# duongve13112002/DiffusionSpatialControl

Measured on AMD Instinct MI355X. Metric: 512x512 images/sec, SD1.5 25-step DPM++2M Karras with region-biased cross-attention, higher is better.
Workload: dtype f16; 1 GPU; SD1.5 512x512, 25-step DPM++2M Karras, CFG 7.5, 2 region masks, 1 image(s) per generation, 2 generation(s) in flight per GPU; images_per_gpu=1, parallelism=dp1 (independent images, no per-step collective), hip_graph=True, outputs_finite=True, full=False

## Files before the change

### diffusionspatialcontrol_amd/_lib.py

```python
import ctypes
import os
import re

_HERE = os.path.dirname(os.path.abspath(__file__))
_LIB = None


class DscLibraryError(RuntimeError):
    pass


def lib_path():
    return os.environ.get("DSC_LIB_PATH") or os.path.join(_HERE, "libdsc_hip.so")


def header_path():
    return os.path.join(os.path.dirname(_HERE), "include", "dsc_hip.h")


def declared_symbols():
    txt = open(header_path()).read()
    txt = re.sub(r"/\*.*?\*/", "", txt, flags=re.S)
    return sorted(set(re.findall(r"\b(dsc_[a-z0-9_]+)\s*\(", txt)))

# ... 34 lines not shown
    "dsc_cfg_linear_step_rows": (ctypes.c_int, [_vp, _vp, _vp, ctypes.c_int, _vp, _vp, _vp, _vp, ctypes.c_int, ctypes.c_int,
                                 _vp, ctypes.c_int, ctypes.c_int, ctypes.c_int, _vp]),
    "dsc_cfg_linear_step_rows_rescale": (ctypes.c_int, [_vp, _vp, _vp, ctypes.c_int, _vp, _vp, _vp, _vp, ctypes.c_int,
                                         ctypes.c_int, _vp, _vp, ctypes.c_int, ctypes.c_int, ctypes.c_int, _vp]),
    "dsc_dpmpp2m_update": (ctypes.c_int, [_vp, _vp, _vp] + [ctypes.c_float] * 3 + [_vp, ctypes.c_int64, ctypes.c_int, _vp]),
    "dsc_groupnorm_workspace_bytes": (ctypes.c_size_t, [ctypes.c_int] * 4),
    "dsc_groupnorm_silu": (ctypes.c_int, [_vp] * 4 + [ctypes.c_int] * 4 + [ctypes.c_float, ctypes.c_int, ctypes.c_int,
                                                                             _vp, ctypes.c_size_t, _vp]),
    "dsc_groupnorm_nhwc_workspace_bytes": (ctypes.c_size_t, [ctypes.c_int] * 4),
    "dsc_debug_set_gn_mode": (None, [ctypes.c_int]),
    "dsc_groupnorm_silu_nhwc": (ctypes.c_int, [_vp] * 5 + [ctypes.c_int64] + [ctypes.c_int] * 4 +
                                [ctypes.c_float, ctypes.c_int, ctypes.c_int, _vp, ctypes.c_size_t, _vp]),
    "dsc_groupnorm_silu_nhwc_cat": (ctypes.c_int, [_vp, _vp, ctypes.c_int] + [_vp] * 5 + [ctypes.c_int64] + [ctypes.c_int] * 4 +
                                    [ctypes.c_float, ctypes.c_int, ctypes.c_int, _vp, ctypes.c_size_t, _vp]),
    "dsc_set_workspace_slot": (ctypes.c_int, [ctypes.c_int]),
    "dsc_set_tuning_profile": (ctypes.c_int, [ctypes.c_int]),
    "dsc_get_tuning_profile": (ctypes.c_int, []),
    "dsc_linear_lt_stats": (None, [_vp]),
    "dsc_has_library_gemm": (ctypes.c_int, []),
    "dsc_add_bias_residual": (ctypes.c_int, [_vp] * 4 + [ctypes.c_int64, ctypes.c_int, ctypes.c_int, _vp]),
    "dsc_linear_f16": (ctypes.c_int, [_vp] * 5 + [ctypes.c_int64, ctypes.c_int, ctypes.c_int] + [ctypes.c_int64] * 3 +
                       [ctypes.c_int, ctypes.c_int, _vp]),
    "dsc_debug_set_conv_stamps": (None, [_vp]),
    "dsc_debug_set_conv_ring": (None, [ctypes.c_int]),
    "dsc_conv3x3_supported": (ctypes.c_int, [ctypes.c_int] * 5),
    "dsc_conv3x3_workspace_bytes": (ctypes.c_size_t, [ctypes.c_int] * 6),
    "dsc_conv3x3_nhwc_f16": (ctypes.c_int, [_vp] * 5 + [ctypes.c_int] * 5 + [ctypes.c_int64] * 3 +
                             [ctypes.c_int, ctypes.c_int, ctypes.c_int, ctypes.c_int, _vp, ctypes.c_size_t, _vp]),
    "dsc_conv3x3_up2x_pack_f16": (ctypes.c_int, [_vp, _vp, ctypes.c_int, ctypes.c_int, _vp]),
    "dsc_conv3x3_up2x_supported": (ctypes.c_int, [ctypes.c_int] * 5),
    "dsc_conv3x3_up2x_workspace_bytes": (ctypes.c_size_t, [ctypes.c_int] * 6),
    "dsc_conv3x3_up2x_nhwc_f16": (ctypes.c_int, [_vp] * 4 + [ctypes.c_int] * 6 + [_vp, ctypes.c_size_t, ctypes.c_int64, ctypes.c_int64,
                                                                                   ctypes.c_int, _vp]),
    "dsc_conv3x3_fewcin_f16": (ctypes.c_int, [_vp] * 4 + [ctypes.c_int] * 6 + [_vp]),
    "dsc_linear_lt_f16": (ctypes.c_int, [_vp] * 5 + [ctypes.c_int64, ctypes.c_int, ctypes.c_int] + [ctypes.c_int64] * 3 +
                          [ctypes.c_int, _vp]),
    "dsc_linear_rows_f16": (ctypes.c_int, [_vp] * 4 + [ctypes.c_int] * 3 + [ctypes.c_int64] * 2 + [ctypes.c_int, ctypes.c_int, _vp]),
    "dsc_linear_ln_f16": (ctypes.c_int, [_vp] * 5 + [ctypes.c_int64, ctypes.c_int, ctypes.c_int] + [ctypes.c_int64] * 3 +
                          [ctypes.c_int, _vp, ctypes.c_int, _vp, ctypes.c_float, _vp, ctypes.c_int, _vp]),
    "dsc_debug_set_gemm_stages": (None, [ctypes.c_int]),
    "dsc_linear_qkv_f16": (ctypes.c_int, [_vp] * 5 + [ctypes.c_int64, ctypes.c_int, ctypes.c_int, ctypes.c_int64, ctypes.c_int64,
                                          ctypes.c_int, ctypes.c_int, _vp, ctypes.c_int, _vp, ctypes.c_float, ctypes.c_int, _vp]),
    "dsc_add_layernorm": (ctypes.c_int, [_vp] * 6 + [ctypes.c_int64, ctypes.c_int, ctypes.c_float, ctypes.c_int, _vp]),
    "dsc_geglu": (ctypes.c_int, [_vp, _vp, ctypes.c_int64, ctypes.c_int, ctypes.c_int, _vp]),
    "dsc_linear_splitk_workspace_bytes": (ctypes.c_size_t, [ctypes.c_int64, ctypes.c_int, ctypes.c_int, ctypes.c_int]),
    "dsc_linear_splitk_f16": (ctypes.c_int, [_vp] * 5 + [ctypes.c_int64, ctypes.c_int, ctypes.c_int] + [ctypes.c_int64] * 3 +
                              [ctypes.c_int, _vp, ctypes.c_size_t, ctypes.c_int, _vp]),
    "dsc_conv3x3_gn_rows": (ctypes.c_int, [ctypes.c_int] * 7),
    "dsc_conv3x3_gn_nhwc_f16": (ctypes.c_int, [_vp] * 4 + [ctypes.c_int64, _vp, _vp] + [ctypes.c_int] * 5 + [ctypes.c_int64] * 3 +
                                [ctypes.c_int, _vp, ctypes.c_int, ctypes.c_int, _vp]),
    "dsc_linear_gn_rows": (ctypes.c_int, [ctypes.c_int64, ctypes.c_int, ctypes.c_int, ctypes.c_int, ctypes.c_int]),
    "dsc_linear_gn_f16": (ctypes.c_int, [_vp] * 5 + [ctypes.c_int64, ctypes.c_int, ctypes.c_int] + [ctypes.c_int64] * 3 +
                          [ctypes.c_int, _vp, ctypes.c_int, ctypes.c_int, _vp]),
    "dsc_groupnorm_apply_nhwc": (ctypes.c_int, [_vp] * 5 + [ctypes.c_int] * 5 + [ctypes.c_float, ctypes.c_int, ctypes.c_int, _vp]),
    "dsc_softmax_rows_f16": (ctypes.c_int, [_vp, _vp, ctypes.c_int64, ctypes.c_int, ctypes.c_int64, ctypes.c_int64, ctypes.c_float,
                                            ctypes.c_int, _vp]),
    "dsc_latent_resample_noise": (ctypes.c_int, [_vp] * 3 + [ctypes.c_int] * 6 + [_vp] * 4 + [ctypes.c_float, _vp]),
    "dsc_ip_xattn_add_f16": (ctypes.c_int, [_vp] + [ctypes.c_longlong] * 3 + [_vp, _vp, ctypes.c_longlong, _vp, _vp] +
                             [ctypes.c_int] * 5 + [ctypes.c_float, _vp]),
}


def load_library():
    global _LIB
    if _LIB is not None:
        return _LIB
# ... 40 lines not shown
```

### diffusionspatialcontrol_amd/csrc/conv3x3.hip

```cpp
#include "dsc_common.h"
#include "dsc_hip.h"
#include "gn_partials.h"
#include <type_traits>

extern int g_dsc_tuning_profile;

namespace {

constexpr int BM = 128, BN = 64, BK = 64, T = 256;
constexpr int kBStageBytes = BN * BK * 2;
constexpr int kAPiecesMax = 25;
constexpr int kABytes = kAPiecesMax * 1024;
constexpr int kRingOff = 0;
constexpr int a_off(int S) { return S * kBStageBytes; }
constexpr int pad_off(int S) { return a_off(S) + 2 * kABytes; }
constexpr int lds_bytes(int S) { return pad_off(S) + 1024; }
constexpr int a_bytes(int NT, int TW) { return NT == 4 && TW == 16 ? 23 * 1024 : kABytes; }
constexpr int lds_bytes_up2x(int TW) { return a_off(4) + 2 * a_bytes(4, TW) + 1024; }
constexpr int kEpiStride = BN + 4;
constexpr unsigned kOob = 0x80000000u;

struct ConvParams {
    const half_t* x; const half_t* w; const half_t* bias; const half_t* res; half_t* out; float* ws;
    int B, H, W, Cin, Cout;
// ... 31 lines not shown
template <int S, int NT>
constexpr int younger_dmas(int t) {
    int n = 0;
    for (int i = 1; i <= S - 2; ++i) n += ((t - i) % NT + NT) % NT == 0 ? 9 : 2;
    return n;
}
template <int S, int NT>
__device__ __forceinline__ void wait_step(int t) {
    switch (t) {
        case 0: wait_vm<younger_dmas<S, NT>(0)>(); break;
        case 1: wait_vm<younger_dmas<S, NT>(1)>(); break;
        case 2: wait_vm<younger_dmas<S, NT>(2)>(); break;
        case 3: wait_vm<younger_dmas<S, NT>(3)>(); break;
        case 4: wait_vm<younger_dmas<S, NT>(4)>(); break;
        case 5: wait_vm<younger_dmas<S, NT>(5)>(); break;
        case 6: wait_vm<younger_dmas<S, NT>(6)>(); break;
        case 7: wait_vm<younger_dmas<S, NT>(7)>(); break;
        default: wait_vm<younger_dmas<S, NT>(8)>(); break;
    }
}

template <int TW>
__device__ __forceinline__ int halo_swz(int hy, int hx) {
    if constexpr (TW == 16) return (hx >> 1) & 7;
    else return ((hx >> 1) ^ ((hy & 1) << 2)) & 7;
}

struct Frags { h8_t w[4], x0[4], x1[4]; };

__device__ __forceinline__ h8_t lds_read(unsigned byte_addr) {
    return *reinterpret_cast<const __attribute__((address_space(3))) h8_t*>((uintptr_t)byte_addr);
}

template <int TW, int S, int NLOAD, int NT>
__device__ __forceinline__ void conv3x3_body(const ConvParams& p) {
    static_assert(NT == 9 || NT == 4, "nine taps, or the four of a phase of the 2x-upsampled form");
    static_assert(NT % S == 0, "the ring depth must divide the taps of a slice (a tile's stage is its tap % S)");
    static_assert(NLOAD == 0 || NLOAD == 4, "loader waves mirror the four computing waves' DMA shares");
    static_assert(NT == 9 || NLOAD == 0, "the phase form has no loader-wave variant");
    constexpr bool LOADER = NLOAD > 0;
    constexpr bool UP = NT == 4;
    constexpr int kAB = a_bytes(NT, TW);
    constexpr int kAOff = a_off(S), kPadOff = kAOff + 2 * kAB;
    constexpr int NSB = 16 / TW;
    constexpr int HWD = TW + 2;
    constexpr int HS = 10 * HWD;
    constexpr int NSLOT = NSB * HS;
    constexpr int NPIECE = (NSLOT + 7) / 8;
    constexpr int NPAR = TW == 16 ? 1 : 2;
    constexpr int MT1 = (32 / TW) * HWD * 128;
    static_assert(NPIECE * 1024 <= kAB && NPIECE <= 28, "halo does not fit");

    extern __shared__ __attribute__((aligned(16))) char smem[];

    const int lane = threadIdx.x & 63, wave_all = __builtin_amdgcn_readfirstlane(threadIdx.x >> 6);
    const bool is_loader = LOADER && wave_all >= 4;
    const int wave = wave_all & 3;
    const int r = lane & 31, hh = lane >> 5;
    const int wm = wave >> 1, wn = wave & 1;

    const int total = p.mt * p.nt * p.splits;
    const int per = gridDim.x >> 3;
    const int v = (blockIdx.x & 7) * per + (blockIdx.x >> 3);
    if (v >= total) return;
    long long st0 = 0, st1 = 0, st2 = 0, sc0 = 0, sc1 = 0, sc2 = 0;
    if (p.stamps) { st0 = __builtin_amdgcn_s_memrealtime(); sc0 = __builtin_amdgcn_s_memtime(); }
    int bm, bn, sp;
    if (p.order) {
        const int rest = fdiv(v, p.fd_nt);
        bn = v - rest * p.nt;
        sp = fdiv(rest, p.fd_mt); bm = rest - sp * p.mt;
    } else {
        const int rest = fdiv(v, p.fd_mt);
        bm = v - rest * p.mt;
        sp = fdiv(rest, p.fd_nt); bn = rest - sp * p.nt;
    }
    const int n0 = bn * BN;
    const int cb = sp * p.cps, ce = min(p.nc, cb + p.cps);
    const int ns = (ce - cb) * NT;
    int phase = 0;
    if constexpr (UP) {
        const int mts = p.mt >> 2;
        phase = (bm >= mts) + (bm >= 2 * mts) + (bm >= 3 * mts);
        bm -= phase * mts;
    }
    const int PY = phase >> 1, PX = phase & 1;

    const __amdgpu_buffer_rsrc_t xr = __builtin_amdgcn_make_buffer_rsrc(const_cast<half_t*>(p.x), 0, p.x_bytes, 0x00020000);
    const __amdgpu_buffer_rsrc_t wr = __builtin_amdgcn_make_buffer_rsrc(const_cast<half_t*>(p.w), 0, p.w_bytes, 0x00020000);

    unsigned wvoff[2];
#pragma unroll
    for (int pc = 0; pc < 2; ++pc) {
        const int row = (pc * 4 + wave) * 8 + (lane >> 3);
        const int chunk = (lane & 7) ^ ((row >> 1) & 7);
        wvoff[pc] = ((unsigned)(phase * p.Cout + n0 + row) * (unsigned)NT * (unsigned)p.Cin + chunk * 8) * 2u;
    }
    auto issue_b = [&](unsigned soff, int stage) {
#pragma unroll
        for (int pc = 0; pc < 2; ++pc) dma16(wr, wvoff[pc], soff, kRingOff + stage * kBStageBytes + (pc * 4 + wave) * 1024);
    };
    auto tile_soff = [&](int c, int t) { return ((unsigned)t * (unsigned)p.Cin + (unsigned)c * BK) * 2u; };

    const bool dma_wave = !LOADER || is_loader;
    if (dma_wave) {
#pragma unroll
        for (int k = 0; k < S; ++k) issue_b(tile_soff(cb, k), k);
    }

    int ob[NSB], oy[NSB], ox[NSB];
#pragma unroll
    for (int sb = 0; sb < NSB; ++sb) {
        const int g = bm * NSB + sb;
        const int b = fdiv(g, p.fd_bpi), r2 = g - b * p.bpi, byy = fdiv(r2, p.fd_bpr);
        ob[sb] = g < p.nblk ? b : -1;
        oy[sb] = byy * 8; ox[sb] = (r2 - byy * p.bpr) * TW;
    }
    unsigned aoff[7];
#pragma unroll
    for (int i = 0; i < 7; ++i) {
        const int slot = (i * 4 + wave) * 8 + (lane >> 3);
        unsigned off = kOob;
        if (slot < NSLOT) {
            const int sb = slot / HS, rem = slot % HS;
            const int hy = rem / HWD, hx = rem % HWD;
            const int b = NSB == 1 ? ob[0] : (sb ? ob[NSB - 1] : ob[0]);
            const int y = (NSB == 1 ? oy[0] : (sb ? oy[NSB - 1] : oy[0])) - 1 + hy;
            const int x = (NSB == 1 ? ox[0] : (sb ? ox[NSB - 1] : ox[0])) - 1 + hx;
            if (b >= 0 && y >= 0 && y < p.H && x >= 0 && x < p.W) {
                const int px = p.up ? (b * p.sh + (y >> 1)) * p.sw + (x >> 1) : (b * p.H + y) * p.W + x;
                off = ((unsigned)px * (unsigned)p.ldx + (((lane & 7) ^ halo_swz<TW>(hy, hx)) << 3)) * 2u;
            }
        }
        aoff[i] = off;
    }
    auto issue_a = [&](int i, int c, int ab) {
        const int piece = i * 4 + wave;
        const unsigned dst = piece < NPIECE ? kAOff + ab * kAB + piece * 1024 : kPadOff;
        dma16(xr, aoff[i], (unsigned)c * (BK * 2), dst);
    };
    constexpr int NDX = UP ? 2 : 3;
    unsigned xaddr[NPAR][NDX][4], waddr[4], waddr_hi[4];
    {
        const int m = wm * 64 + r;
        const int sb = m / (8 * TW), py = (m % (8 * TW)) / TW + PY, pxl = m % TW + PX;
        const int slot00 = sb * HS + py * HWD + pxl;
#pragma unroll
        for (int par = 0; par < NPAR; ++par)
#pragma unroll
            for (int dx = 0; dx < NDX; ++dx) {
                const int sw = halo_swz<TW>(py + par, pxl + dx);
#pragma unroll
                for (int ks = 0; ks < 4; ++ks) xaddr[par][dx][ks] = (unsigned)(kAOff + (slot00 + dx) * 128 + (((2 * ks + hh) ^ sw) << 4));
            }
        const int wrow = wn * 32 + r;
#pragma unroll
        for (int ks = 0; ks < 4; ++ks) {
            waddr[ks] = (unsigned)(kRingOff + wrow * 128 + (((2 * ks + hh) ^ ((wrow >> 1) & 7)) << 4));
            waddr_hi[ks] = waddr[ks] + 4 * kBStageBytes;
        }
    }
    auto load_frags = [&](Frags& f, int ab, int t) {
        const int dy = t / NDX, dx = t % NDX;
        const unsigned abase = ab * kAB + dy * HWD * 128;
        const int stg = t % S;
#pragma unroll
        for (int ks = 0; ks < 4; ++ks) {
            f.w[ks] = stg < 4 ? lds_read(waddr[ks] + stg * kBStageBytes) : lds_read(waddr_hi[ks] + (stg - 4) * kBStageBytes);
            f.x0[ks] = lds_read(xaddr[NPAR == 1 ? 0 : (dy & 1)][dx][ks] + abase);
            f.x1[ks] = lds_read(xaddr[NPAR == 1 ? 0 : (dy & 1)][dx][ks] + abase + MT1);
        }
    };

    f16x_t acc[2];
// ... 154 lines not shown
                        if (p.res) v += (float)p.res[gp * p.ldr + c];
                        if (p.nchw) p.out[((long long)b * p.Cout + c) * hw + pin] = (half_t)v;
                        else p.out[gp * p.ldo + c] = (half_t)v;
                    }
                }
            }
        }
    }
    if (p.gn_part) {
        float* dst = ob[0] >= 0 ? p.gn_part + ((long long)ob[0] * p.bpi + (bm - ob[0] * p.bpi)) * p.gn_G * 4 : nullptr;
        dsc_gn::gn_tile_partials(gs, gq, reinterpret_cast<float*>(smem) + BM * kEpiStride, n0, p.gn_cpg, p.gn_G, dst);
    }
    if (p.stamps && threadIdx.x == 0) {
        unsigned hwid;
        asm volatile("s_getreg_b32 %0, hwreg(HW_REG_HW_ID)" : "=s"(hwid));
        unsigned xcc;
        asm volatile("s_getreg_b32 %0, hwreg(HW_REG_XCC_ID)" : "=s"(xcc));
        long long* o = p.stamps + (long long)v * 8;
        o[0] = st0; o[1] = st1; o[2] = st2; o[3] = __builtin_amdgcn_s_memrealtime();
        o[4] = sc1 - sc0; o[5] = sc2 - sc1; o[6] = __builtin_amdgcn_s_memtime() - sc2; o[7] = ((long long)xcc << 32) | hwid;
    }
}

template <int TW, int S, int NLOAD = 0>
__global__ __launch_bounds__(T + 64 * NLOAD, (S == 3 || NLOAD ? 2 : 1)) void conv3x3_kernel(ConvParams p) {
    conv3x3_body<TW, S, NLOAD, 9>(p);
}

template <int TW>
__global__ __launch_bounds__(T, (TW == 16 ? 2 : 1)) void conv3x3_kernel_up2x(ConvParams p) {
    conv3x3_body<TW, 4, 0, 4>(p);
}

__global__ __launch_bounds__(256) void conv3x3_reduce(ConvParams p) {
    const int cv = p.Cout >> 3;
    const int idx = blockIdx.x * 256 + threadIdx.x;
    if (idx >= (int)p.onpix * cv) return;
    const int gpi = fdiv(idx, p.fd_cv);
    const long long gp = gpi;
    const int n = (idx - gpi * cv) * 8;
    float s[8] = {0, 0, 0, 0, 0, 0, 0, 0};
    for (int k = 0; k < p.splits; ++k) {
        const float* src = p.ws + ((long long)k * p.onpix + gp) * p.Cout + n;
        const f4x_t a = *reinterpret_cast<const f4x_t*>(src), b = *reinterpret_cast<const f4x_t*>(src + 4);
#pragma unroll
        for (int j = 0; j < 4; ++j) { s[j] += a[j]; s[4 + j] += b[j]; }
    }
    h8_t bv = {0, 0, 0, 0, 0, 0, 0, 0}, rv = {0, 0, 0, 0, 0, 0, 0, 0};
    if (p.bias) bv = *reinterpret_cast<const h8_t*>(p.bias + n);
    if (p.res) rv = *reinterpret_cast<const h8_t*>(p.res + gp * p.ldr + n);
    h8_t o;
#pragma unroll
    for (int j = 0; j < 8; ++j) o[j] = (half_t)(s[j] + (float)bv[j] + (float)rv[j]);
    *reinterpret_cast<h8_t*>(p.out + gp * p.ldo + n) = o;
}

long long* g_conv_stamps = nullptr;
int g_conv_ring = 0;

bool al16(const void* q) { return (reinterpret_cast<uintptr_t>(q) & 15) == 0; }

int tile_width(int H, int W) {
    if (H < 1 || W < 1) return 0;
    if (W % 16 == 0) return 16;
    if (W % 8 == 0) return 8;
    return ((W + 15) / 16 * 16 - W <= (W + 7) / 8 * 8 - W) ? 16 : 8;
}

int g_conv_loaders = 1;
int g_conv_order = -1;
double g_conv_small_step = 0.14;
double g_up2x_small_step = 0.14;
int auto_splits(int tiles, int nc, long long npix, int cout, int taps, int per_cu) {
    int best = 1;
    double best_t = 1e30;
    for (int s = 1; s <= nc; ++s) {
        if (nc % s != 0) continue;
        const long long wgs = (long long)tiles * s;
        if (s > 1 && wgs > 1024) break;
        const double small = (taps == 4 ? g_up2x_small_step : g_conv_small_step) / 0.26;
        const double load = wgs <= 256 ? small : (per_cu == 1 ? small * (double)((wgs + 255) / 256)
                                                              : (wgs <= 512 ? 1.15 : 1.15 * (double)wgs / 512.0));
        double t = (double)taps * nc / s * 0.26 * load + 5.0;
        if (s > 1) t += 4.0 + (double)s * (double)npix * cout * 8.0 / 3.0e6;
        if (t < best_t) { best_t = t; best = s; }
    }
    return best;
}

size_t split_ws_bytes(const ConvParams& p, long long pixels) {
    return p.splits > 1 ? (size_t)p.splits * pixels * p.Cout * sizeof(float) : 0;
}

int plan(int B, int H, int W, int Cin, int Cout, int splits, int resample, long long ldx, long long ldr, long long ldo, int taps,
         ConvParams* p) {
    const int tw = tile_width(H, W);
    if (!tw || Cin % BK != 0 || Cout <= 0 || resample < 0 || resample > DSC_CONV_UPSAMPLE_CEIL) return 0;
    p->B = B; p->H = H; p->W = W; p->Cin = Cin; p->Cout = Cout;
    p->ldx = ldx; p->ldr = ldr; p->ldo = ldo;
    const bool ceil = resample == DSC_CONV_UPSAMPLE_CEIL;
    p->up = resample == DSC_CONV_UPSAMPLE2X || ceil ? 1 : 0;
    p->sh = ceil ? (H + 1) / 2 : H / 2; p->sw = ceil ? (W + 1) / 2 : W / 2;
    p->sub2 = resample == DSC_CONV_STRIDE2 ? 1 : (resample == DSC_CONV_STRIDE2_PAD_BR ? 2 : 0);
    p->oh = (H + 1) / 2; p->ow = (W + 1) / 2;
    p->nc = Cin / BK;
    p->bpr = (W + tw - 1) / tw; p->bpi = ((H + 7) / 8) * p->bpr; p->nblk = B * p->bpi;
    const int nsb = 16 / tw;
    p->mt = (p->nblk + nsb - 1) / nsb; p->nt = (Cout + BN - 1) / BN;
    if (taps == 4) p->mt *= 4;
    p->npix = (long long)B * H * W;
    const long long computed = taps == 4 ? 4 * p->npix : p->npix;
    p->onpix = p->sub2 ? (long long)B * p->oh * p->ow : computed;
    if (Cout % BN != 0) splits = 1;
    if (splits <= 0) splits = auto_splits(p->mt * p->nt, p->nc, computed, Cout, taps, taps == 4 && tw == 8 ? 1 : 2);
    if (splits > p->nc) splits = p->nc;
    p->cps = (p->nc + splits - 1) / splits;
    p->splits = (p->nc + p->cps - 1) / p->cps;
    const long long total = (long long)p->mt * p->nt * p->splits;
    p->fd_mt = make_fastdiv(p->mt, total); p->fd_nt = make_fastdiv(p->nt, total);
    p->fd_bpi = make_fastdiv(p->bpi, (long long)p->mt * nsb + nsb); p->fd_bpr = make_fastdiv(p->bpr, p->bpi);
    p->order = g_conv_order >= 0 ? g_conv_order : (computed >= 2ll * Cout ? 1 : 0);
    const long long in_pix = p->up ? (long long)B * p->sh * p->sw : p->npix;
    p->x_bytes = (unsigned)(((in_pix - 1) * ldx + Cin) * 2);
    p->w_bytes = (unsigned)((taps == 4 ? 16ll : 9ll) * Cin * Cout * 2);
    return tw;
}

int check_operands(const void* x, const void* w, const void* bias, const void* residual, const void* out, int B, int H, int W, int Cin,
                   int Cout, long long ldx, long long ldr, long long ldo, int out_nchw, int dtype, int taps) {
    if (!x || !w || !out || B <= 0 || H <= 0 || W <= 0 || Cin <= 0 || Cout <= 0) return DSC_ERR_BAD_ARG;
    if (dtype != DSC_F16) return DSC_ERR_UNSUPPORTED;
    if (ldx < Cin || (!out_nchw && ldo < Cout) || (residual && ldr < Cout)) return DSC_ERR_BAD_ARG;
    if (ldx % 8 != 0 || (Cout % 8 == 0 && !out_nchw && ldo % 8 != 0) || (residual && Cout % 8 == 0 && ldr % 8 != 0)) return DSC_ERR_UNSUPPORTED;
    if (!al16(x) || !al16(w) || !al16(out) || (bias && !al16(bias)) || (residual && !al16(residual))) return DSC_ERR_UNSUPPORTED;
    if ((taps == 4 ? 4ll : 1ll) * B * H * W * (ldx > ldo ? ldx : ldo) >= (1ll << 30) ||
        (taps == 4 ? 16ll : 9ll) * Cin * Cout >= (1ll << 30)) return DSC_ERR_UNSUPPORTED;
    return DSC_OK;
}

int bind(ConvParams* p, const void* x, const void* w, const void* bias, const void* residual, void* out, void* workspace,
         size_t workspace_bytes) {
    p->x = static_cast<const half_t*>(x); p->w = static_cast<const half_t*>(w);
    p->bias = static_cast<const half_t*>(bias); p->res = static_cast<const half_t*>(residual);
    p->out = static_cast<half_t*>(out); p->ws = static_cast<float*>(workspace);
    p->stamps = g_conv_stamps;
    if (p->splits > 1 && (!workspace || workspace_bytes < split_ws_bytes(*p, p->onpix) || !al16(workspace))) return DSC_ERR_WORKSPACE;
    return DSC_OK;
}

struct KernelForm { void (*fn)(ConvParams); int lds, block; };
const KernelForm g_forms[] = {
    {conv3x3_kernel<16, 3>, lds_bytes(3), T}, {conv3x3_kernel<8, 3>, lds_bytes(3), T},
    {conv3x3_kernel<16, 9>, lds_bytes(9), T}, {conv3x3_kernel<8, 9>, lds_bytes(9), T},
    {conv3x3_kernel<16, 9, 4>, lds_bytes(9), T + 256}, {conv3x3_kernel<8, 9, 4>, lds_bytes(9), T + 256},
    {conv3x3_kernel_up2x<16>, lds_bytes_up2x(16), T}, {conv3x3_kernel_up2x<8>, lds_bytes_up2x(8), T}};

int launch(const ConvParams& p, int tw, int taps, hipStream_t st) {
    const int total = p.mt * p.nt * p.splits;
    int form = 3;
    if (taps != 4) {
        int ring = g_conv_ring;
        if (ring != 3 && ring != 9) ring = (total <= 256 && g_dsc_tuning_profile == DSC_TUNE_LATENCY) ? 9 : 3;
        const bool loaders = ring == 9 && (g_conv_loaders == 2 || (g_conv_loaders == 1 && tw == 16));
        form = loaders ? 2 : (ring == 9 ? 1 : 0);
    }
    static bool attr_set = false;
    if (!attr_set) {
        for (const KernelForm& f : g_forms) (void)hipFuncSetAttribute(reinterpret_cast<const void*>(f.fn), hipFuncAttributeMaxDynamicSharedMemorySize, 160 * 1024);
        attr_set = true;
    }
    const KernelForm& k = g_forms[2 * form + (tw == 16 ? 0 : 1)];
    DSC_LAUNCH(k.fn, dim3(((total + 7) / 8) * 8), dim3(k.block), (size_t)k.lds, st, p);
    if (hipGetLastError() != hipSuccess) return DSC_ERR_LAUNCH;
    if (p.splits > 1) {
        ConvParams r = p;
        const long long n = p.onpix * (p.Cout / 8);
        r.fd_cv = make_fastdiv(p.Cout / 8, n + 256);
        DSC_LAUNCH(conv3x3_reduce, dim3((unsigned)((n + 255) / 256)), dim3(256), 0, st, r);
        if (hipGetLastError() != hipSuccess) return DSC_ERR_LAUNCH;
    }
    return DSC_OK;
}

struct GnArgs { const void* add; int64_t add_ld; float* part; int groups; };

int conv_impl(const void* x, const void* w, const void* bias, const void* residual, void* out,
              int B, int H, int W, int Cin, int Cout, int64_t ldx, int64_t ldr, int64_t ldo,
              int resample, int out_nchw, int splits, int dtype, void* workspace, size_t workspace_bytes, void* stream,
              const GnArgs* gn) {
    int rc = check_operands(x, w, bias, residual, out, B, H, W, Cin, Cout, ldx, ldr, ldo, out_nchw, dtype, 9);
    if (rc != DSC_OK) return rc;
    const bool stride2 = resample == DSC_CONV_STRIDE2 || resample == DSC_CONV_STRIDE2_PAD_BR;
    if ((stride2 && out_nchw) || (resample == DSC_CONV_STRIDE2_PAD_BR && ((H | W) & 1))) return DSC_ERR_UNSUPPORTED;
    if (out_nchw) splits = 1;
    ConvParams p{};
    const int tw = plan(B, H, W, Cin, Cout, splits, resample, ldx, ldr, ldo, 9, &p);
    if (!tw) return DSC_ERR_UNSUPPORTED;
    p.nchw = out_nchw ? 1 : 0;
    if (gn) {
        p.add = static_cast<const half_t*>(gn->add); p.add_ld = gn->add_ld;
        p.gn_part = gn->part; p.gn_G = gn->groups; p.gn_cpg = Cout / gn->groups;
    }
    rc = bind(&p, x, w, bias, residual, out, workspace, workspace_bytes);
    return rc != DSC_OK ? rc : launch(p, tw, 9, static_cast<hipStream_t>(stream));
}

}

extern "C" void dsc_debug_set_conv_stamps(void* device_buffer) { g_conv_stamps = static_cast<long long*>(device_buffer); }

extern "C" void dsc_debug_set_conv_ring(int stages) {
    if (stages >= 500) g_up2x_small_step = (stages - 500) / 100.0;
    else if (stages >= 400) g_conv_loaders = stages - 400;
    else if (stages >= 300) g_conv_order = stages - 300;
    else if (stages >= 200) g_conv_small_step = (stages - 200) / 100.0;
    else g_conv_ring = stages;
}

extern "C" int dsc_conv3x3_supported(int B, int H, int W, int Cin, int Cout) {
    ConvParams p{};
    if (B <= 0 || H <= 0 || W <= 0 || (long long)B * H * W * (long long)(Cin > Cout ? Cin : Cout) >= (1ll << 30) ||
        9ll * Cin * Cout >= (1ll << 30)) return 0;
    return plan(B, H, W, Cin, Cout, 0, 0, Cin, 0, Cout, 9, &p) ? 1 : 0;
}

extern "C" size_t dsc_conv3x3_workspace_bytes(int B, int H, int W, int Cin, int Cout, int splits) {
    ConvParams p{};
    if (B <= 0 || H <= 0 || W <= 0 || !plan(B, H, W, Cin, Cout, splits, 0, Cin, 0, Cout, 9, &p)) return 0;
    return split_ws_bytes(p, p.npix);
}

extern "C" int dsc_conv3x3_nhwc_f16(const void* x, const void* w, const void* bias, const void* residual, void* out,
                                    int B, int H, int W, int Cin, int Cout, int64_t ldx, int64_t ldr, int64_t ldo,
                                    int resample, int out_nchw, int splits, int dtype, void* workspace,
                                    size_t workspace_bytes, void* stream) {
    return conv_impl(x, w, bias, residual, out, B, H, W, Cin, Cout, ldx, ldr, ldo, resample, out_nchw, splits, dtype, workspace,
                     workspace_bytes, stream, nullptr);
}

extern "C" int dsc_conv3x3_gn_rows(int B, int H, int W, int Cin, int Cout, int groups, int resample) {
    ConvParams p{};
    if (B <= 0 || H <= 0 || W <= 0 || groups <= 0 || Cout % BN != 0 || Cout % groups != 0 || Cout / groups > 64 || Cout / groups < 2) return 0;
    if (resample == DSC_CONV_STRIDE2 || resample == DSC_CONV_STRIDE2_PAD_BR) return 0;
    if (plan(B, H, W, Cin, Cout, 0, resample, Cin, 0, Cout, 9, &p) != 16 || p.splits != 1 || p.bpi > 128) return 0;
    return p.bpi;
// ... 47 lines not shown

}

extern "C" int dsc_conv3x3_up2x_pack_f16(const void* w, void* packed, int Cin, int Cout, void* stream) {
    if (!w || !packed || Cin <= 0 || Cout <= 0) return DSC_ERR_BAD_ARG;
    if (Cin % BK != 0 || 16ll * Cin * Cout >= (1ll << 30) || !al16(w) || !al16(packed)) return DSC_ERR_UNSUPPORTED;
    const long long n = 16ll * Cout * (Cin / 8);
    DSC_LAUNCH(conv3x3_up2x_pack_kernel, dim3((unsigned)((n + 255) / 256)), dim3(256), 0, static_cast<hipStream_t>(stream),
               static_cast<const half_t*>(w), static_cast<half_t*>(packed), Cin, Cout);
    return hipGetLastError() == hipSuccess ? DSC_OK : DSC_ERR_LAUNCH;
}

extern "C" int dsc_conv3x3_up2x_supported(int B, int h, int w, int Cin, int Cout) {
    ConvParams p{};
    return plan_up2x(B, h, w, Cin, Cout, 0, Cin, Cout, &p) ? 1 : 0;
}

extern "C" size_t dsc_conv3x3_up2x_workspace_bytes(int B, int h, int w, int Cin, int Cout, int splits) {
    ConvParams p{};
    return plan_up2x(B, h, w, Cin, Cout, splits, Cin, Cout, &p) ? split_ws_bytes(p, p.onpix) : 0;
}

extern "C" int dsc_conv3x3_up2x_nhwc_f16(const void* x, const void* w_packed, const void* bias, void* out, int B, int h, int w,
                                         int Cin, int Cout, int splits, void* workspace, size_t workspace_bytes, int64_t ldx,
                                         int64_t ldo, int dtype, void* stream) {
    int rc = check_operands(x, w_packed, bias, nullptr, out, B, h, w, Cin, Cout, ldx, 0, ldo, 0, dtype, 4);
    if (rc != DSC_OK) return rc;
    ConvParams p{};
    const int tw = plan_up2x(B, h, w, Cin, Cout, splits, ldx, ldo, &p);
    if (!tw) return DSC_ERR_UNSUPPORTED;
    rc = bind(&p, x, w_packed, bias, nullptr, out, workspace, workspace_bytes);
    return rc != DSC_OK ? rc : launch(p, tw, 4, static_cast<hipStream_t>(stream));
}
```

### diffusionspatialcontrol_amd/modules/u_net_condition_modify.py

```python
import inspect
import math
from dataclasses import dataclass, field
from typing import Any, Dict, Optional, Tuple

import torch
import torch.nn as nn
import torch.nn.functional as F

from .. import ops
from .attention_modify import AttnProcessor, AttnProcessor2_0, _IPAdapterProcessor, prepared_ip_rows


class ImageProjection(nn.Module):

    def __init__(self, image_embed_dim=768, cross_attention_dim=768, num_image_text_embeds=32):
        super().__init__()
        self.num_image_text_embeds = num_image_text_embeds
        self.image_embeds = nn.Linear(image_embed_dim, num_image_text_embeds * cross_attention_dim)
        self.norm = nn.LayerNorm(cross_attention_dim)

    def forward(self, image_embeds):
        b = image_embeds.shape[0]
        return self.norm(self.image_embeds(image_embeds).reshape(b, self.num_image_text_embeds, -1))

# ... 463 lines not shown
                        lambda: (self.time_emb_proj.bias + self.conv1.bias).contiguous())

    def forward(self, x, temb_act, temb_add=None):
        if isinstance(x, tuple):
            h, x = self.norm1.of_cat(*x)
        else:
            h = self.norm1(x)
        if temb_add is None:
            temb_add = F.linear(temb_act, self.time_emb_proj.weight, self.temb_bias())
        g = self.norm2.num_groups
        fuse = h.is_cuda and h.dtype == torch.float16 and h.shape[0] * h.shape[2] * h.shape[3] >= GN_FUSE_MIN_ROWS
        if fuse and ops.conv3x3_gn_rows(h, self.conv1.weight, g) > 0:
            h = self.norm2(ops.conv3x3_gn(h, self.conv1.weight, g, add=temb_add[:h.shape[0]]))
        else:
            h = self.norm2(_conv3x3(h, self.conv1.weight), add=temb_add)
        if self.conv_shortcut is None:
            if fuse and ops.conv3x3_gn_rows(h, self.conv2.weight, g) > 0:
                return ops.conv3x3_gn(h, self.conv2.weight, g, bias=self.conv2.bias, residual=x)
            return _conv3x3(h, self.conv2.weight, self.conv2.bias, residual=x)
        h = _conv3x3(h, self.conv2.weight)
        b = _derived(self, "sb", (self.conv_shortcut.bias, self.conv2.bias),
                     lambda: (self.conv_shortcut.bias + self.conv2.bias).contiguous())
        bsz, _, hh, ww = h.shape
        t, part = self.conv_shortcut.tokens(_tokens(x), bias=b, residual=_tokens(h), gn_groups=g)
        return _with_gn(_image(t, hh, ww), part)


class Downsample2D(nn.Module):
    def __init__(self, c):
        super().__init__()
        self.conv = nn.Conv2d(c, c, 3, stride=2, padding=1)

    def forward(self, x):
        y = ops.conv3x3_try(x, self.conv.weight, self.conv.bias, mode=ops.CONV_STRIDE2)
        return self.conv(x) if y is None else y


class Upsample2D(nn.Module):
    def __init__(self, c):
        super().__init__()
        self.conv = nn.Conv2d(c, c, 3, padding=1)

    def forward(self, x, output_size=None):
        if output_size is not None:
            output_size = tuple(int(v) for v in output_size)
        w = self.conv.weight
        if output_size in (None, (2 * x.shape[2], 2 * x.shape[3])) and ops.USE_UP2X_PHASES and ops.conv3x3_up2x_supported(x, w):
            return ops.conv3x3_up2x(x, _derived(self, "up2x", (w,), lambda: ops.conv3x3_up2x_pack(w)), self.conv.bias)
        if output_size is None:
            y = ops.conv3x3_try(x, w, self.conv.bias, mode=ops.CONV_UPSAMPLE2X)
            return self.conv(F.interpolate(x, scale_factor=2.0, mode="nearest")) if y is None else y
        y = None
        if all(t in (2 * s_, 2 * s_ - 1) for t, s_ in zip(output_size, x.shape[2:])):
            y = ops.conv3x3_try(x, w, self.conv.bias, mode=ops.CONV_UPSAMPLE_SIZE, size=output_size)
        return self.conv(F.interpolate(x, size=output_size, mode="nearest")) if y is None else y


class _Block(nn.Module):

    def __init__(self, res_io, temb_dim, cfg, heads, depth, down=False, up=False):
        super().__init__()
        cout = res_io[-1][1]
        self.resnets = nn.ModuleList([ResnetBlock2D(i, o, temb_dim, cfg.norm_num_groups, cfg.norm_eps) for i, o in res_io])
        self.has_attn = depth > 0
        if self.has_attn:
            self.attentions = nn.ModuleList([
# ... 270 lines not shown
```

### diffusionspatialcontrol_amd/ops.py

```python
import ctypes
import os

import numpy as np
import torch

from . import _lib

FLAG_REF_FP16_ROUNDING = 1
FLAG_BIAS_IS_FINAL = 2
FLAG_REUSE_STATS = 4
FLAG_ROWS_PADDED = 256
FLAG_SIGMA_PER_GROUP = 512
REGION_ROW_STRIDE = 100

def _stream_ptr(t):
    return ctypes.c_void_p(torch.cuda.current_stream(t.device).cuda_stream)


def _p(t):
    return ctypes.c_void_p(t.data_ptr()) if t is not None else None


def _i64x3(a, b, c):
    return (ctypes.c_int64 * 3)(a, b, c)
# ... 786 lines not shown


def conv3x3_up2x_supported(x, weight):
    if not (USE_DSC_CONV and x.is_cuda and x.dtype == torch.float16 and weight.dtype == torch.float16 and x.dim() == 4
            and weight.dim() == 4 and tuple(weight.shape[2:]) == (3, 3) and weight.shape[1] == x.shape[1]):
        return False
    B, C, h, w = x.shape
    return bool(_lib.load_library().dsc_conv3x3_up2x_supported(B, h, w, C, weight.shape[0]))


def conv3x3_up2x(x, packed, bias=None, splits=0):
    if x.dim() != 4 or x.dtype != torch.float16:
        raise ValueError("conv3x3_up2x: x must be a [B, Cin, h, w] fp16 tensor")
    B, Cin, h, w = x.shape
    if (packed.dim() != 4 or packed.shape[0] != 4 or packed.shape[2] != 4 or packed.shape[3] != Cin
            or packed.dtype != torch.float16 or not packed.is_contiguous()):
        raise ValueError(f"conv3x3_up2x: packed must be the contiguous fp16 [4, Cout, 4, {Cin}] tensor of conv3x3_up2x_pack, "
                         f"not {tuple(packed.shape)}")
    Cout = packed.shape[1]
    if bias is not None and (bias.dtype != torch.float16 or bias.numel() != Cout or not bias.is_contiguous()):
        raise ValueError("conv3x3_up2x: bias must be a contiguous fp16 [Cout] tensor")
    _require_gpu(x, packed)
    lib = _lib.load_library()
    x, _, _, _ = _conv3x3_operands("conv3x3_up2x", x, None, None, None)
    out = torch.empty((B, Cout, 2 * h, 2 * w), dtype=x.dtype, device=x.device, memory_format=torch.channels_last)
    nbytes = lib.dsc_conv3x3_up2x_workspace_bytes(B, h, w, Cin, Cout, splits)
    ws = _workspace(x.device, nbytes) if nbytes else None
    rc = lib.dsc_conv3x3_up2x_nhwc_f16(_p(x), _p(packed), _p(bias), _p(out), B, h, w, Cin, Cout, splits, _p(ws),
                                       ws.numel() * 8 if ws is not None else 0, Cin, Cout, 0, _stream_ptr(x))
    _lib.check(rc, "dsc_conv3x3_up2x_nhwc_f16")
    return out


def conv3x3_fewcin(x, weight_t, bias, cout):
    _require_gpu(x, weight_t)
    x = x.contiguous()
    B, Cin, H, W = x.shape
    out = torch.empty((B, cout, H, W), dtype=x.dtype, device=x.device, memory_format=torch.channels_last)
    rc = _lib.load_library().dsc_conv3x3_fewcin_f16(_p(x), _p(weight_t), _p(bias), _p(out), B, Cin, H, W, cout, 0, _stream_ptr(x))
    _lib.check(rc, "dsc_conv3x3_fewcin_f16")
    return out


def linear_rows(x, weight, bias=None, silu_out=False, sinusoid_dim=0):
    _require_gpu(x, weight)
    N, K = weight.shape
    if sinusoid_dim:
        if x.dtype != torch.float32 or x.dim() != 1 or sinusoid_dim != K:
            raise ValueError("linear_rows: sinusoid input is an fp32 [M] tensor and sinusoid_dim == weight.shape[1]")
        x = x.contiguous()
        M, ldx = x.shape[0], 0
    else:
        x = x if x.stride(-1) == 1 else x.contiguous()
        M, ldx = x.shape[0], x.stride(0)
    out = torch.empty((M, N), dtype=weight.dtype, device=weight.device)
    flags = (1 if sinusoid_dim else 0) | (2 if silu_out else 0)
    rc = _lib.load_library().dsc_linear_rows_f16(_p(x), _p(weight), _p(bias), _p(out), M, N, K, ldx, N, flags, 0, _stream_ptr(weight))
    _lib.check(rc, "dsc_linear_rows_f16")
    return out


def add_bias_residual(a, b, bias=None):
    _require_gpu(a, b)
    if a.dim() == 4:
        cl = torch.channels_last
        if not a.is_contiguous(memory_format=cl):
# ... 268 lines not shown
```

### include/dsc_hip.h

```cpp
#ifndef DSC_HIP_H
#define DSC_HIP_H

#include <stddef.h>
#include <stdint.h>

#ifdef __cplusplus
extern "C" {
#endif

#define DSC_OK                0
#define DSC_ERR_BAD_ARG      -1
#define DSC_ERR_UNSUPPORTED  -2
#define DSC_ERR_WORKSPACE    -3
#define DSC_ERR_LAUNCH       -4

#define DSC_F16 0
#define DSC_FLAG_REF_FP16_ROUNDING 1u
#define DSC_FLAG_REUSE_STATS       4u
#define DSC_FLAG_ROWS_PADDED     256u
#define DSC_FLAG_BIAS_IS_FINAL     2u
#define DSC_FLAG_SIGMA_PER_GROUP 512u

int dsc_abi_version(void);
const char* dsc_target_arch(void);
// ... 104 lines not shown
                            int B, int C, int hw, int groups, float eps, int apply_silu, int dtype,
                            void* workspace, size_t workspace_bytes, void* stream);
int dsc_groupnorm_silu_nhwc_cat(const void* x1, const void* x2, int C1, void* cat, void* y, const void* gamma,
                                const void* beta, const void* add, int64_t add_row_stride, int B, int C, int hw,
                                int groups, float eps, int apply_silu, int dtype, void* workspace, size_t workspace_bytes,
                                void* stream);

int dsc_add_bias_residual(const void* a, const void* b, const void* bias, void* out, int64_t rows, int C,
                          int dtype, void* stream);

int dsc_linear_f16(const void* x, const void* w, const void* bias, const void* residual, void* out,
                   int64_t M, int N, int K, int64_t ldx, int64_t ldr, int64_t ldo, int geglu, int dtype, void* stream);

#define DSC_CONV_UPSAMPLE2X 1
#define DSC_CONV_STRIDE2 2
#define DSC_CONV_STRIDE2_PAD_BR 3
#define DSC_CONV_UPSAMPLE_CEIL 4
int dsc_conv3x3_supported(int B, int H, int W, int Cin, int Cout);
void dsc_debug_set_conv_stamps(void* device_buffer);
void dsc_debug_set_conv_ring(int stages);
size_t dsc_conv3x3_workspace_bytes(int B, int H, int W, int Cin, int Cout, int splits);
int dsc_conv3x3_nhwc_f16(const void* x, const void* w, const void* bias, const void* residual, void* out,
                         int B, int H, int W, int Cin, int Cout, int64_t ldx, int64_t ldr, int64_t ldo,
                         int resample, int out_nchw, int splits, int dtype, void* workspace, size_t workspace_bytes,
                         void* stream);

int dsc_conv3x3_up2x_pack_f16(const void* w, void* packed, int Cin, int Cout, void* stream);
int dsc_conv3x3_up2x_supported(int B, int h, int w, int Cin, int Cout);
size_t dsc_conv3x3_up2x_workspace_bytes(int B, int h, int w, int Cin, int Cout, int splits);
int dsc_conv3x3_up2x_nhwc_f16(const void* x, const void* w_packed, const void* bias, void* out, int B, int h, int w,
                              int Cin, int Cout, int splits, void* workspace, size_t workspace_bytes, int64_t ldx,
                              int64_t ldo, int dtype, void* stream);

int dsc_linear_ln_f16(const void* x, const void* w, const void* bias, const void* residual, void* out,
                      int64_t M, int N, int K, int64_t ldx, int64_t ldr, int64_t ldo, int geglu,
                      const float* ln_in, int ln_nb, const float* ln_cvec, float ln_eps, float* ln_out,
                      int dtype, void* stream);
void dsc_debug_set_gemm_stages(int stages);
int dsc_linear_qkv_f16(const void* x, const void* w, const void* bias, void* q_out, void* kv_out,
                       int64_t M, int C, int K, int64_t ldx, int64_t ldq, int heads, int seq_len,
                       const float* ln_in, int ln_nb, const float* ln_cvec, float ln_eps, int dtype, void* stream);

int dsc_conv3x3_fewcin_f16(const void* x_nchw, const void* w_t, const void* bias, void* out_nhwc,
                           int B, int Cin, int H, int W, int Cout, int dtype, void* stream);

int dsc_linear_lt_f16(const void* x, const void* w, const void* bias, const void* residual, void* out,
                      int64_t M, int N, int K, int64_t ldx, int64_t ldr, int64_t ldo, int dtype, void* stream);
int dsc_has_library_gemm(void);
int dsc_set_workspace_slot(int slot);
#define DSC_TUNE_LATENCY 0
#define DSC_TUNE_THROUGHPUT 1
int dsc_set_tuning_profile(int profile);
int dsc_get_tuning_profile(void);
void dsc_linear_lt_stats(long long out[3]);

#define DSC_ROWS_SINUSOID_IN 1
#define DSC_ROWS_SILU_OUT 2
int dsc_linear_rows_f16(const void* x, const void* w, const void* bias, void* out, int M, int N, int K,
                        int64_t ldx, int64_t ldo, int flags, int dtype, void* stream);

int dsc_add_layernorm(const void* x, const void* a, const void* gamma, const void* beta, void* sum_out, void* y,
                      int64_t rows, int C, float eps, int dtype, void* stream);

int dsc_geglu(const void* x, void* y, int64_t rows, int n, int dtype, void* stream);

int dsc_conv3x3_gn_rows(int B, int H, int W, int Cin, int Cout, int groups, int resample);
// ... 33 lines not shown
```

Before: 11.77 images/s.

## Add polyphase stride-2 conv3x3 kernel for UNet downsample layers

Adds a down2x form of the implicit-GEMM conv3x3 kernel. It splits the stride-2 input into four polyphase sub-images so each output tile computes only the outputs it keeps, with taps that fall into padding fed by zero weight tiles. The UNet Downsample forward uses it by default. The previous stride-2 path may have computed or loaded redundant work. This adds a new kernel instantiation, split heuristics and index math that could mishandle edges or cost occupancy.

```diff
diff --git a/diffusionspatialcontrol_amd/_lib.py b/diffusionspatialcontrol_amd/_lib.py
--- a/diffusionspatialcontrol_amd/_lib.py
+++ b/diffusionspatialcontrol_amd/_lib.py
@@ -90,6 +90,10 @@
     "dsc_conv3x3_up2x_workspace_bytes": (ctypes.c_size_t, [ctypes.c_int] * 6),
     "dsc_conv3x3_up2x_nhwc_f16": (ctypes.c_int, [_vp] * 4 + [ctypes.c_int] * 6 + [_vp, ctypes.c_size_t, ctypes.c_int64, ctypes.c_int64,
                                                                                    ctypes.c_int, _vp]),
+    "dsc_conv3x3_down2x_supported": (ctypes.c_int, [ctypes.c_int] * 5),
+    "dsc_conv3x3_down2x_workspace_bytes": (ctypes.c_size_t, [ctypes.c_int] * 6),
+    "dsc_conv3x3_down2x_nhwc_f16": (ctypes.c_int, [_vp] * 4 + [ctypes.c_int] * 6 + [_vp, ctypes.c_size_t, ctypes.c_int64, ctypes.c_int64,
+                                                                                     ctypes.c_int, _vp]),
     "dsc_conv3x3_fewcin_f16": (ctypes.c_int, [_vp] * 4 + [ctypes.c_int] * 6 + [_vp]),
     "dsc_linear_lt_f16": (ctypes.c_int, [_vp] * 5 + [ctypes.c_int64, ctypes.c_int, ctypes.c_int] + [ctypes.c_int64] * 3 +
                           [ctypes.c_int, _vp]),
diff --git a/diffusionspatialcontrol_amd/csrc/conv3x3.hip b/diffusionspatialcontrol_amd/csrc/conv3x3.hip
--- a/diffusionspatialcontrol_amd/csrc/conv3x3.hip
+++ b/diffusionspatialcontrol_amd/csrc/conv3x3.hip
@@ -87,14 +87,15 @@
     return *reinterpret_cast<const __attribute__((address_space(3))) h8_t*>((uintptr_t)byte_addr);
 }
 
-template <int TW, int S, int NLOAD, int NT>
+template <int TW, int S, int NLOAD, int NT, bool DN = false>
 __device__ __forceinline__ void conv3x3_body(const ConvParams& p) {
-    static_assert(NT == 9 || NT == 4, "nine taps, or the four of a phase of the 2x-upsampled form");
+    static_assert(NT == 9 || NT == 4, "nine taps, or the four of a phase of the 2x-upsampled / the stride-2 form");
+    static_assert(!DN || NT == 4, "the stride-2 phase form has four taps per virtual slice");
     static_assert(NT % S == 0, "the ring depth must divide the taps of a slice (a tile's stage is its tap % S)");
     static_assert(NLOAD == 0 || NLOAD == 4, "loader waves mirror the four computing waves' DMA shares");
     static_assert(NT == 9 || NLOAD == 0, "the phase form has no loader-wave variant");
     constexpr bool LOADER = NLOAD > 0;
-    constexpr bool UP = NT == 4;
+    constexpr bool UP = NT == 4 && !DN;
     constexpr int kAB = a_bytes(NT, TW);
     constexpr int kAOff = a_off(S), kPadOff = kAOff + 2 * kAB;
     constexpr int NSB = 16 / TW;
@@ -149,13 +150,25 @@
     for (int pc = 0; pc < 2; ++pc) {
         const int row = (pc * 4 + wave) * 8 + (lane >> 3);
         const int chunk = (lane & 7) ^ ((row >> 1) & 7);
-        wvoff[pc] = ((unsigned)(phase * p.Cout + n0 + row) * (unsigned)NT * (unsigned)p.Cin + chunk * 8) * 2u;
-    }
+        wvoff[pc] = ((unsigned)(phase * p.Cout + n0 + row) * (unsigned)(DN ? 9 : NT) * (unsigned)p.Cin + chunk * 8) * 2u;
+    }
+    constexpr unsigned kZeroTile = 0xffffffffu;
     auto issue_b = [&](unsigned soff, int stage) {
-#pragma unroll
-        for (int pc = 0; pc < 2; ++pc) dma16(wr, wvoff[pc], soff, kRingOff + stage * kBStageBytes + (pc * 4 + wave) * 1024);
+        const bool zero = DN && soff == kZeroTile;
+#pragma unroll
+        for (int pc = 0; pc < 2; ++pc)
+            dma16(wr, zero ? kOob : wvoff[pc], zero ? 0u : soff, kRingOff + stage * kBStageBytes + (pc * 4 + wave) * 1024);
     };
-    auto tile_soff = [&](int c, int t) { return ((unsigned)t * (unsigned)p.Cin + (unsigned)c * BK) * 2u; };
+    auto tile_soff = [&](int c, int t) -> unsigned {
+        if constexpr (DN) {
+            const int q = c & 3, a = t >> 1, b = t & 1;
+            const int dy = (q >> 1) ? 2 * a : 2 * a - 1, dx = (q & 1) ? 2 * b : 2 * b - 1;
+            if (dy < 0 || dx < 0) return kZeroTile;
+            return ((unsigned)(3 * dy + dx) * (unsigned)p.Cin + (unsigned)(c >> 2) * BK) * 2u;
+        } else {
+            return ((unsigned)t * (unsigned)p.Cin + (unsigned)c * BK) * 2u;
+        }
+    };
 
     const bool dma_wave = !LOADER || is_loader;
     if (dma_wave) {
@@ -183,7 +196,8 @@
             const int y = (NSB == 1 ? oy[0] : (sb ? oy[NSB - 1] : oy[0])) - 1 + hy;
             const int x = (NSB == 1 ? ox[0] : (sb ? ox[NSB - 1] : ox[0])) - 1 + hx;
             if (b >= 0 && y >= 0 && y < p.H && x >= 0 && x < p.W) {
-                const int px = p.up ? (b * p.sh + (y >> 1)) * p.sw + (x >> 1) : (b * p.H + y) * p.W + x;
+                const int px = DN ? (b * p.sh + 2 * y) * p.sw + 2 * x
+                                  : (p.up ? (b * p.sh + (y >> 1)) * p.sw + (x >> 1) : (b * p.H + y) * p.W + x);
                 off = ((unsigned)px * (unsigned)p.ldx + (((lane & 7) ^ halo_swz<TW>(hy, hx)) << 3)) * 2u;
             }
         }
@@ -192,9 +206,11 @@
     auto issue_a = [&](int i, int c, int ab) {
         const int piece = i * 4 + wave;
         const unsigned dst = piece < NPIECE ? kAOff + ab * kAB + piece * 1024 : kPadOff;
-        dma16(xr, aoff[i], (unsigned)c * (BK * 2), dst);
+        unsigned soff = (unsigned)c * (BK * 2);
+        if constexpr (DN) soff = (unsigned)(c >> 2) * (BK * 2) + (unsigned)(((c >> 1) & 1) * p.sw + (c & 1)) * (unsigned)p.ldx * 2u;
+        dma16(xr, aoff[i], soff, dst);
     };
-    constexpr int NDX = UP ? 2 : 3;
+    constexpr int NDX = NT == 4 ? 2 : 3;
     unsigned xaddr[NPAR][NDX][4], waddr[4], waddr_hi[4];
     {
         const int m = wm * 64 + r;
@@ -415,6 +431,11 @@
     conv3x3_body<TW, 4, 0, 4>(p);
 }
 
+template <int TW>
+__global__ __launch_bounds__(T, (TW == 16 ? 2 : 1)) void conv3x3_kernel_down2x(ConvParams p) {
+    conv3x3_body<TW, 4, 0, 4, true>(p);
+}
+
 __global__ __launch_bounds__(256) void conv3x3_reduce(ConvParams p) {
     const int cv = p.Cout >> 3;
     const int idx = blockIdx.x * 256 + threadIdx.x;
@@ -454,14 +475,15 @@
 int g_conv_order = -1;
 double g_conv_small_step = 0.14;
 double g_up2x_small_step = 0.14;
-int auto_splits(int tiles, int nc, long long npix, int cout, int taps, int per_cu) {
+double g_down2x_small_step = 0.14;
+int auto_splits(int tiles, int nc, long long npix, int cout, int taps, int per_cu, bool down = false) {
     int best = 1;
     double best_t = 1e30;
     for (int s = 1; s <= nc; ++s) {
         if (nc % s != 0) continue;
         const long long wgs = (long long)tiles * s;
         if (s > 1 && wgs > 1024) break;
-        const double small = (taps == 4 ? g_up2x_small_step : g_conv_small_step) / 0.26;
+        const double small = (down ? g_down2x_small_step : (taps == 4 ? g_up2x_small_step : g_conv_small_step)) / 0.26;
         const double load = wgs <= 256 ? small : (per_cu == 1 ? small * (double)((wgs + 255) / 256)
                                                               : (wgs <= 512 ? 1.15 : 1.15 * (double)wgs / 512.0));
         double t = (double)taps * nc / s * 0.26 * load + 5.0;
@@ -476,7 +498,9 @@
 }
 
 int plan(int B, int H, int W, int Cin, int Cout, int splits, int resample, long long ldx, long long ldr, long long ldo, int taps,
-         ConvParams* p) {
+         ConvParams* p, int in_h = 0, int in_w = 0) {
+    const bool down = in_h > 0;
+    const bool up4 = taps == 4 && !down;
     const int tw = tile_width(H, W);
     if (!tw || Cin % BK != 0 || Cout <= 0 || resample < 0 || resample > DSC_CONV_UPSAMPLE_CEIL) return 0;
     p->B = B; p->H = H; p->W = W; p->Cin = Cin; p->Cout = Cout;
@@ -484,18 +508,19 @@
     const bool ceil = resample == DSC_CONV_UPSAMPLE_CEIL;
     p->up = resample == DSC_CONV_UPSAMPLE2X || ceil ? 1 : 0;
     p->sh = ceil ? (H + 1) / 2 : H / 2; p->sw = ceil ? (W + 1) / 2 : W / 2;
+    if (down) { p->sh = in_h; p->sw = in_w; }
     p->sub2 = resample == DSC_CONV_STRIDE2 ? 1 : (resample == DSC_CONV_STRIDE2_PAD_BR ? 2 : 0);
     p->oh = (H + 1) / 2; p->ow = (W + 1) / 2;
-    p->nc = Cin / BK;
+    p->nc = (down ? 4 : 1) * (Cin / BK);
     p->bpr = (W + tw - 1) / tw; p->bpi = ((H + 7) / 8) * p->bpr; p->nblk = B * p->bpi;
     const int nsb = 16 / tw;
     p->mt = (p->nblk + nsb - 1) / nsb; p->nt = (Cout + BN - 1) / BN;
-    if (taps == 4) p->mt *= 4;
+    if (up4) p->mt *= 4;
     p->npix = (long long)B * H * W;
-    const long long computed = taps == 4 ? 4 * p->npix : p->npix;
+    const long long computed = up4 ? 4 * p->npix : p->npix;
     p->onpix = p->sub2 ? (long long)B * p->oh * p->ow : computed;
     if (Cout % BN != 0) splits = 1;
-    if (splits <= 0) splits = auto_splits(p->mt * p->nt, p->nc, computed, Cout, taps, taps == 4 && tw == 8 ? 1 : 2);
+    if (splits <= 0) splits = auto_splits(p->mt * p->nt, p->nc, computed, Cout, taps, taps == 4 && tw == 8 ? 1 : 2, down);
     if (splits > p->nc) splits = p->nc;
     p->cps = (p->nc + splits - 1) / splits;
     p->splits = (p->nc + p->cps - 1) / p->cps;
@@ -503,9 +528,9 @@
     p->fd_mt = make_fastdiv(p->mt, total); p->fd_nt = make_fastdiv(p->nt, total);
     p->fd_bpi = make_fastdiv(p->bpi, (long long)p->mt * nsb + nsb); p->fd_bpr = make_fastdiv(p->bpr, p->bpi);
     p->order = g_conv_order >= 0 ? g_conv_order : (computed >= 2ll * Cout ? 1 : 0);
-    const long long in_pix = p->up ? (long long)B * p->sh * p->sw : p->npix;
+    const long long in_pix = p->up || down ? (long long)B * p->sh * p->sw : p->npix;
     p->x_bytes = (unsigned)(((in_pix - 1) * ldx + Cin) * 2);
-    p->w_bytes = (unsigned)((taps == 4 ? 16ll : 9ll) * Cin * Cout * 2);
+    p->w_bytes = (unsigned)((up4 ? 16ll : 9ll) * Cin * Cout * 2);
     return tw;
 }
 
@@ -536,11 +561,12 @@
     {conv3x3_kernel<16, 3>, lds_bytes(3), T}, {conv3x3_kernel<8, 3>, lds_bytes(3), T},
     {conv3x3_kernel<16, 9>, lds_bytes(9), T}, {conv3x3_kernel<8, 9>, lds_bytes(9), T},
     {conv3x3_kernel<16, 9, 4>, lds_bytes(9), T + 256}, {conv3x3_kernel<8, 9, 4>, lds_bytes(9), T + 256},
-    {conv3x3_kernel_up2x<16>, lds_bytes_up2x(16), T}, {conv3x3_kernel_up2x<8>, lds_bytes_up2x(8), T}};
-
-int launch(const ConvParams& p, int tw, int taps, hipStream_t st) {
+    {conv3x3_kernel_up2x<16>, lds_bytes_up2x(16), T}, {conv3x3_kernel_up2x<8>, lds_bytes_up2x(8), T},
+    {conv3x3_kernel_down2x<16>, lds_bytes_up2x(16), T}, {conv3x3_kernel_down2x<8>, lds_bytes_up2x(8), T}};
+
+int launch(const ConvParams& p, int tw, int taps, hipStream_t st, bool down = false) {
     const int total = p.mt * p.nt * p.splits;
-    int form = 3;
+    int form = down ? 4 : 3;
     if (taps != 4) {
         int ring = g_conv_ring;
         if (ring != 3 && ring != 9) ring = (total <= 256 && g_dsc_tuning_profile == DSC_TUNE_LATENCY) ? 9 : 3;
@@ -593,7 +619,8 @@
 extern "C" void dsc_debug_set_conv_stamps(void* device_buffer) { g_conv_stamps = static_cast<long long*>(device_buffer); }
 
 extern "C" void dsc_debug_set_conv_ring(int stages) {
-    if (stages >= 500) g_up2x_small_step = (stages - 500) / 100.0;
+    if (stages >= 600) g_down2x_small_step = (stages - 600) / 100.0;
+    else if (stages >= 500) g_up2x_small_step = (stages - 500) / 100.0;
     else if (stages >= 400) g_conv_loaders = stages - 400;
     else if (stages >= 300) g_conv_order = stages - 300;
     else if (stages >= 200) g_conv_small_step = (stages - 200) / 100.0;
@@ -707,3 +734,36 @@
     rc = bind(&p, x, w_packed, bias, nullptr, out, workspace, workspace_bytes);
     return rc != DSC_OK ? rc : launch(p, tw, 4, static_cast<hipStream_t>(stream));
 }
+
+
+namespace {
+
+int plan_down2x(int B, int H, int W, int Cin, int Cout, int splits, long long ldx, long long ldo, ConvParams* p) {
+    if (B <= 0 || H <= 0 || W <= 0 || Cin <= 0 || Cout <= 0 || ((H | W) & 1) || Cin % BK != 0 || Cout % BN != 0) return 0;
+    if ((long long)B * H * W * (long long)(Cin > Cout ? Cin : Cout) >= (1ll << 30) || 9ll * Cin * Cout >= (1ll << 30)) return 0;
+    return plan(B, H / 2, W / 2, Cin, Cout, splits, 0, ldx, 0, ldo, 4, p, H, W);
+}
+
+}
+
+extern "C" int dsc_conv3x3_down2x_supported(int B, int H, int W, int Cin, int Cout) {
+    ConvParams p{};
+    return plan_down2x(B, H, W, Cin, Cout, 0, Cin, Cout, &p) ? 1 : 0;
+}
+
+extern "C" size_t dsc_conv3x3_down2x_workspace_bytes(int B, int H, int W, int Cin, int Cout, int splits) {
+    ConvParams p{};
+    return plan_down2x(B, H, W, Cin, Cout, splits, Cin, Cout, &p) ? split_ws_bytes(p, p.onpix) : 0;
+}
+
+extern "C" int dsc_conv3x3_down2x_nhwc_f16(const void* x, const void* w, const void* bias, void* out, int B, int H, int W,
+                                           int Cin, int Cout, int splits, void* workspace, size_t workspace_bytes, int64_t ldx,
+                                           int64_t ldo, int dtype, void* stream) {
+    int rc = check_operands(x, w, bias, nullptr, out, B, H, W, Cin, Cout, ldx, 0, ldo, 0, dtype, 9);
+    if (rc != DSC_OK) return rc;
+    ConvParams p{};
+    const int tw = plan_down2x(B, H, W, Cin, Cout, splits, ldx, ldo, &p);
+    if (!tw) return DSC_ERR_UNSUPPORTED;
+    rc = bind(&p, x, w, bias, nullptr, out, workspace, workspace_bytes);
+    return rc != DSC_OK ? rc : launch(p, tw, 4, static_cast<hipStream_t>(stream), true);
+}
diff --git a/diffusionspatialcontrol_amd/modules/u_net_condition_modify.py b/diffusionspatialcontrol_amd/modules/u_net_condition_modify.py
--- a/diffusionspatialcontrol_amd/modules/u_net_condition_modify.py
+++ b/diffusionspatialcontrol_amd/modules/u_net_condition_modify.py
@@ -519,6 +519,9 @@
         self.conv = nn.Conv2d(c, c, 3, stride=2, padding=1)
 
     def forward(self, x):
+        w = self.conv.weight
+        if ops.USE_DOWN2X_PHASES and ops.conv3x3_down2x_supported(x, w):
+            return ops.conv3x3_down2x(x, w, self.conv.bias)
         y = ops.conv3x3_try(x, self.conv.weight, self.conv.bias, mode=ops.CONV_STRIDE2)
         return self.conv(x) if y is None else y
 
diff --git a/diffusionspatialcontrol_amd/ops.py b/diffusionspatialcontrol_amd/ops.py
--- a/diffusionspatialcontrol_amd/ops.py
+++ b/diffusionspatialcontrol_amd/ops.py
@@ -842,6 +842,40 @@
     return out
 
 
+USE_DOWN2X_PHASES = os.environ.get("DSC_DOWN2X_PHASES", "1") != "0"
+
+
+def conv3x3_down2x_supported(x, weight):
+    if not (USE_DSC_CONV and x.is_cuda and x.dtype == torch.float16 and weight.dtype == torch.float16 and x.dim() == 4
+            and weight.dim() == 4 and tuple(weight.shape[2:]) == (3, 3) and weight.shape[1] == x.shape[1]):
+        return False
+    B, C, H, W = x.shape
+    return bool(_lib.load_library().dsc_conv3x3_down2x_supported(B, H, W, C, weight.shape[0]))
+
+
+def conv3x3_down2x(x, weight, bias=None, splits=0):
+    if x.dim() != 4 or x.dtype != torch.float16:
+        raise ValueError("conv3x3_down2x: x must be a [B, Cin, H, W] fp16 tensor")
+    B, Cin, H, W = x.shape
+    if weight.dim() != 4 or tuple(weight.shape[1:]) != (Cin, 3, 3) or weight.dtype != torch.float16:
+        raise ValueError(f"conv3x3_down2x: weight must be a [Cout, {Cin}, 3, 3] fp16 tensor, not {tuple(weight.shape)}")
+    Cout = weight.shape[0]
+    if bias is not None and (bias.dtype != torch.float16 or bias.numel() != Cout or not bias.is_contiguous()):
+        raise ValueError("conv3x3_down2x: bias must be a contiguous fp16 [Cout] tensor")
+    if H % 2 or W % 2:
+        raise ValueError("conv3x3_down2x: H and W must be even; conv3x3(stride2_ceil=True) takes any side")
+    _require_gpu(x, weight)
+    lib = _lib.load_library()
+    x, weight, _, _ = _conv3x3_operands("conv3x3_down2x", x, weight, None, None)
+    out = torch.empty((B, Cout, H // 2, W // 2), dtype=x.dtype, device=x.device, memory_format=torch.channels_last)
+    nbytes = lib.dsc_conv3x3_down2x_workspace_bytes(B, H, W, Cin, Cout, splits)
+    ws = _workspace(x.device, nbytes) if nbytes else None
+    rc = lib.dsc_conv3x3_down2x_nhwc_f16(_p(x), _p(weight), _p(bias), _p(out), B, H, W, Cin, Cout, splits, _p(ws),
+                                         ws.numel() * 8 if ws is not None else 0, Cin, Cout, 0, _stream_ptr(x))
+    _lib.check(rc, "dsc_conv3x3_down2x_nhwc_f16")
+    return out
+
+
 def conv3x3_fewcin(x, weight_t, bias, cout):
     _require_gpu(x, weight_t)
     x = x.contiguous()
diff --git a/include/dsc_hip.h b/include/dsc_hip.h
--- a/include/dsc_hip.h
+++ b/include/dsc_hip.h
@@ -160,6 +160,12 @@
                               int Cin, int Cout, int splits, void* workspace, size_t workspace_bytes, int64_t ldx,
                               int64_t ldo, int dtype, void* stream);
 
+int dsc_conv3x3_down2x_supported(int B, int H, int W, int Cin, int Cout);
+size_t dsc_conv3x3_down2x_workspace_bytes(int B, int H, int W, int Cin, int Cout, int splits);
+int dsc_conv3x3_down2x_nhwc_f16(const void* x, const void* w, const void* bias, void* out, int B, int H, int W,
+                                int Cin, int Cout, int splits, void* workspace, size_t workspace_bytes, int64_t ldx,
+                                int64_t ldo, int dtype, void* stream);
+
 int dsc_linear_ln_f16(const void* x, const void* w, const void* bias, const void* residual, void* out,
                       int64_t M, int N, int K, int64_t ldx, int64_t ldr, int64_t ldo, int geglu,
                       const float* ln_in, int ln_nb, const float* ln_cvec, float ln_eps, float* ln_out,
```

Result: no change. 11.85 images/s, median of 6 (+0.7%).
